# amberxie88/latent_diffusion_planning

Measured on AMD Instinct MI355X. Metric: latent plans/sec (horizon=9, 100 DDIM steps), higher is better.
Workload: dtype f32; 1 GPU; configs[1]: rm_lift planner ConditionalUnet1D (D=25, T=8, down_dims [256,512,1024]), 100-step DDIM, batch 256 synthetic latents per GPU, random-init weights, Philox noise, hipGraph-captured loop; plans_per_gpu=256, denoise_steps=100, sampler=ddim, graph=True, parallelism=dp1, ranks_seen_by_backend=1, backend=none, range_fallback=0, fp16_plane_launches=0

## Files before the change

### latent_diffusion_planning_amd/csrc/tconv.hpp

```cpp
#pragma once
#include <hip/hip_runtime.h>
#include <stdint.h>
#include <type_traits>

#pragma clang fp contract(off)

#ifndef LDP_W_NT
#define LDP_W_NT 0
#endif
#ifndef LDP_SPLIT_NPROD
#define LDP_SPLIT_NPROD 6
#endif
#ifndef LDP_S16_LF
#define LDP_S16_LF 100
#endif
#ifndef LDP_F16_MINW
#define LDP_F16_MINW 2
#endif
#ifndef LDP_RANGE_GUARD
#define LDP_RANGE_GUARD 1
#endif
#ifndef LDP_KERNARG_TOUCH
#define LDP_KERNARG_TOUCH 1
#endif
#ifndef LDP_KERNARG_PRELOAD
#define LDP_KERNARG_PRELOAD 1
#endif

namespace ldp {

typedef float f32x4 __attribute__((ext_vector_type(4)));

enum : int { MODE_K5 = 0, MODE_DOWN = 1, MODE_UP = 2, MODE_P1 = 3,
             MODE_K3H = 4,
             MODE_K3S = 5 };

enum : int {
  EP_GN = 1,
  EP_FILM = 2,
  EP_RESIN = 4,
  EP_RELU = 8,
  EP_STEP = 16,
  EP_EPSOUT = 32,
};

struct StepCoef {
  float t, inv_sqrt_ab, sqrt_1mab, c_x0, c_x, c_eps, sigma, pad;
};

constexpr int KW_MAX = 8;

struct ConvArgs {
  const float* xa;
  const float* xb;
  int ca, cb;
  const float* w;
  const float* bias;
  const float* bres;
  float* res_out;
  const float* gn_scale;
  const float* gn_bias;
  const float* film_t;
  const float* film_g;
  int film_stride;
  const int* k_dev;
  int k;
  const float* res_in;
  float* out;
  int B, cout, flags;
  int d_real;
  int rows_valid;
  StepCoef coef;
  const float* noise;
  const uint64_t* seed;
  int step;
  float* eps_out;
  int dbg;
  int cs;
  unsigned long long* xchg;
  int kw;
  unsigned long long* kw_slab;
  int kw_slot;
  const uint64_t* ctl;
  unsigned int* fault;
  int h_out, w_tiles, h_in, w_in;
  int ca_real;
  int by_sample;
  float* stats_part;
  int sb_qs;
  unsigned long long* tl;
};

#ifdef LDP_ABLATE
#define LDP_ABL(bit) ((a.dbg & (bit)) != 0)
#else
#define LDP_ABL(bit) (false)
#endif

#ifdef LDP_TIMELINE
#define LDP_TL(i)                                                                                         \
  do {                                                                                                    \
    if (a.tl) {                                                                                           \
      const unsigned long long t_ = (i) == 0 ? ldp_t_entry : __builtin_amdgcn_s_memtime();                \
      if (lane == 0)                                                                                      \
        a.tl[((size_t)(blockIdx.x + gridDim.x * (blockIdx.y + gridDim.y * blockIdx.z)) * 16 + wave) * 8 + (i)] = t_; \
    }                                                                                                     \
  } while (0)
#else
#define LDP_TL(i) do { } while (0)
#endif

__host__ __device__ constexpr int mode_taps(int mode) {
  return mode == MODE_K5 ? 5 : (mode == MODE_DOWN || mode == MODE_K3H || mode == MODE_K3S) ? 3
       : mode == MODE_UP ? 4 : 1;
}
__host__ __device__ constexpr bool mode_2d(int mode) { return mode == MODE_K3H || mode == MODE_K3S; }
__host__ __device__ constexpr int mode_ti(int mode, int to) {
  return mode == MODE_DOWN ? 2 * to : mode == MODE_UP ? to / 2 : mode == MODE_K3H ? to + 2
       : mode == MODE_K3S ? 2 * to + 2 : to;
}
__host__ __device__ constexpr int tap_src(int mode, int to, int j) {
  if (mode == MODE_K5) return to + j - 2;
  if (mode == MODE_DOWN || mode == MODE_K3S) return 2 * to + j;
  if (mode == MODE_K3H) return to + j;
  if (mode == MODE_UP) {
    const int q = to >> 1;
    if ((to & 1) == 0) return j == 0 ? q - 1 : (j == 2 ? q : -1);
    return j == 1 ? q : (j == 3 ? q + 1 : -1);
  }
  return j == 0 ? to : -1;
}
__host__ __device__ constexpr int tap_dst(int mode, int to_n, int ti, int j) {
  for (int to = 0; to < to_n; ++to)
    if (tap_src(mode, to, j) == ti) return to;
  return -1;
}
__host__ __device__ constexpr bool tap_used(int mode, int to_n, int j) {
  const int ti_n = mode_ti(mode, to_n);
  for (int to = 0; to < to_n; ++to) {
    const int ti = tap_src(mode, to, j);
    if (ti >= 0 && ti < ti_n) return true;
  }
  return false;
}
__host__ __device__ constexpr int valid_pairs(int mode, int to_n) {
  const int ti_n = mode_ti(mode, to_n);
  int n = 0;
  for (int to = 0; to < to_n; ++to)
    for (int j = 0; j < mode_taps(mode); ++j) {
      const int ti = tap_src(mode, to, j);
      if (ti >= 0 && ti < ti_n) ++n;
    }
  return n;
}

__device__ __forceinline__ int swz(int row, int slot) { return slot ^ ((4 - (row >> 2)) & 3); }

#ifndef LDP_EPILOGUE_IEEE
#define LDP_EPILOGUE_IEEE 0
#endif
__device__ __forceinline__ float mish_f(float x) {
#if LDP_EPILOGUE_IEEE
  const float e = expf(fminf(x, 20.0f));
  const float n = e * (e + 2.0f);
  return x * (n / (n + 2.0f));
#else
  const float e = __builtin_amdgcn_exp2f(fminf(x, 20.0f) * 1.4426950408889634f);
  const float n = e * (e + 2.0f);
  return x * (n * __builtin_amdgcn_rcpf(n + 2.0f));
#endif
}

template <int CTRL, int ROW_MASK>
__device__ __forceinline__ float dpp_add(float v) {
  return v + __int_as_float(__builtin_amdgcn_update_dpp(0, __float_as_int(v), CTRL, ROW_MASK, 0xF, false));
}
__device__ __forceinline__ float wave_sum(float v) {
  v = dpp_add<0xB1, 0xF>(v);
  v = dpp_add<0x4E, 0xF>(v);
  v = dpp_add<0x114, 0xF>(v);
  v = dpp_add<0x118, 0xF>(v);
  v = dpp_add<0x142, 0xA>(v);
  v = dpp_add<0x143, 0xC>(v);
  return __int_as_float(__builtin_amdgcn_readlane(__float_as_int(v), 63));
}

__device__ __forceinline__ unsigned long long granule_pack(unsigned int tag, float v) {
  const unsigned int b = __float_as_uint(v);
  return ((unsigned long long)(tag ^ b) << 32) | b;
}
typedef unsigned int u32x4_t __attribute__((ext_vector_type(4)));
constexpr int AUX_SC1 = 16;

__device__ __forceinline__ bool granule_ok(unsigned long long g, unsigned int tag) {
  return ((unsigned int)(g >> 32) ^ (unsigned int)g) == tag;
}

__device__ __forceinline__ void philox4x32_10(uint64_t seed, uint64_t elem, uint32_t step, uint32_t stream,
                                              uint32_t (&out)[4]) {
  uint32_t c0 = (uint32_t)elem, c1 = (uint32_t)(elem >> 32), c2 = step, c3 = stream;
  uint32_t k0 = (uint32_t)seed, k1 = (uint32_t)(seed >> 32);
#pragma unroll
  for (int r = 0; r < 10; ++r) {
    const uint64_t p0 = (uint64_t)0xD2511F53u * c0;
    const uint64_t p1 = (uint64_t)0xCD9E8D57u * c2;
    const uint32_t n0 = (uint32_t)(p1 >> 32) ^ c1 ^ k0;
    const uint32_t n1 = (uint32_t)p1;
    const uint32_t n2 = (uint32_t)(p0 >> 32) ^ c3 ^ k1;
    const uint32_t n3 = (uint32_t)p0;
    c0 = n0; c1 = n1; c2 = n2; c3 = n3;
    k0 += 0x9E3779B9u; k1 += 0xBB67AE85u;
  }
  out[0] = c0; out[1] = c1; out[2] = c2; out[3] = c3;
}

__device__ __forceinline__ float philox_normal(uint64_t seed, uint64_t elem, uint32_t step,
                                               uint32_t stream) {
  uint32_t w[4];
  philox4x32_10(seed, elem, step, stream, w);
  const float u1 = ((float)(w[0] >> 8) + 0.5f) * (1.0f / 16777216.0f);
  const float u2 = ((float)(w[1] >> 8) + 0.5f) * (1.0f / 16777216.0f);
  return sqrtf(-2.0f * logf(u1)) * cosf(6.28318530717958647692f * u2);
}

__host__ __device__ constexpr int mode_flag_mask(int mode) {
  return mode == MODE_K5 ? (EP_GN | EP_FILM | EP_RESIN)
       : mode == MODE_P1 ? (EP_RESIN | EP_RELU | EP_STEP | EP_EPSOUT)
       : mode_2d(mode) ? EP_RESIN : 0;
}
__host__ __device__ constexpr int mode_flag_forced(int mode) { return mode == MODE_K5 ? EP_GN : 0; }

template <int MODE, int TO, int NWN, int KS, int CPI, int MB = 1, int SPLIT = 0>
struct TConvCfg {
  static constexpr int TI = mode_ti(MODE, TO);
  static constexpr int NJ = mode_taps(MODE);
  static constexpr bool S32 = (SPLIT == 1 || SPLIT == 4) && MB == 2;
  static constexpr bool S16 = (SPLIT == 1 && MB == 1) || SPLIT == 2 || SPLIT == 3;
  static constexpr bool F16 = SPLIT == 3 || SPLIT == 4;
  static constexpr int NPL = F16 ? 2 : 3;
  static constexpr int NWC = S32 ? NWN / 2 : NWN;
  static constexpr int NW = NWC * KS;
  static constexpr int NT = 64 * NW;
  static constexpr int BN = 16 * NWN;
  static constexpr int BNP = BN + 4;
  static constexpr int NC = KS * CPI;
  static constexpr int CH_IT = 16 * NC;
  static constexpr int XT = MB * TI * NC * 256 * (SPLIT ? NPL : 2) / 2;
  static constexpr int NLD = (MB * TI * NC * 64) / NT;
  static constexpr int EPI = MB * KS * TO * 16 * BNP;
  static constexpr int TILE_FLOATS = (2 * XT > EPI) ? 2 * XT : EPI;
  static constexpr bool STATS = MODE == MODE_K3H && BN == 64 && MB == 1 && (NW == 8 || NW == 4);
  static constexpr int LDS_FLOATS = TILE_FLOATS + (STATS ? 2 * NW * 64 : 0);
  static constexpr int LDS_BYTES = LDS_FLOATS * 4;
  static constexpr int EPL = (TO * BN) / 64;
  static_assert((MB * TI * NC * 64) % NT == 0, "staging loads must divide evenly");
  static_assert((TO * BN) % 64 == 0, "epilogue needs TO*BN multiple of 64");
  static_assert(NW <= 16, "at most 16 waves");
  static_assert(!SPLIT || (S32 && MODE == MODE_K5 && NWN % 2 == 0) || (S16 && (MODE == MODE_K5 || MODE == MODE_DOWN || MODE == MODE_UP || ((MODE == MODE_K3S || MODE == MODE_K3H) && SPLIT == 3 && MB == 1)) && MB <= 2 && CPI % 2 == 0),
                "split operands: 32-sample x 32-column wave tiles (SPLIT = 1, MB = 2, k = 5) or 16 x 16 tiles over 32-channel steps (MB = 1, or SPLIT = 2 with MB = 2; k = 5, stride-2, transposed)");
};

struct ConvHot {
  static __host__ __device__ int pack(const ConvArgs& a, bool zfold) {
    return (a.cs & 15) | ((a.kw & 15) << 4) | ((a.by_sample & 1) << 8) | ((a.sb_qs & 15) << 9) | ((zfold ? 1 : 0) << 13) | (((a.by_sample >> 1) & 1) << 14);
  }
};
#if LDP_KERNARG_PRELOAD
#define LDP_KERNEL_PARAMS const float* h_xa, const float* h_xb, const float* h_w, int h_B, int h_ca, int h_cb, int h_cout, \
                          int h_ca_real, int h_pk, int h_dbg, const ConvArgs a_in
#define LDP_KERNEL_ARGS(a, zfold) (a).xa, (a).xb, (a).w, (a).B, (a).ca, (a).cb, (a).cout, (a).ca_real, ConvHot::pack(a, zfold), (a).dbg, (a)
#else
#define LDP_KERNEL_PARAMS const ConvArgs a
#define LDP_KERNEL_ARGS(a, zfold) (a)
#endif

typedef __bf16 bf16x8_t __attribute__((ext_vector_type(8)));
typedef float f32x16 __attribute__((ext_vector_type(16)));
__device__ __forceinline__ void split4(const f32x4 v, uint2& h, uint2& m, uint2& l) {
  unsigned short hh[4], mm[4], ll[4];
#pragma unroll
  for (int i = 0; i < 4; ++i) {
    const __bf16 bh = (__bf16)v[i];
    const float r1 = v[i] - (float)bh;
    const __bf16 bm = (__bf16)r1;
    const float r2 = r1 - (float)bm;
    const __bf16 bl = (__bf16)r2;
    hh[i] = __builtin_bit_cast(unsigned short, bh); mm[i] = __builtin_bit_cast(unsigned short, bm); ll[i] = __builtin_bit_cast(unsigned short, bl);
  }
  h = uint2{(unsigned)hh[0] | ((unsigned)hh[1] << 16), (unsigned)hh[2] | ((unsigned)hh[3] << 16)};
  m = uint2{(unsigned)mm[0] | ((unsigned)mm[1] << 16), (unsigned)mm[2] | ((unsigned)mm[3] << 16)};
  l = uint2{(unsigned)ll[0] | ((unsigned)ll[1] << 16), (unsigned)ll[2] | ((unsigned)ll[3] << 16)};
}

typedef _Float16 f16x8_t __attribute__((ext_vector_type(8)));
__device__ __forceinline__ void split4h(const f32x4 v, uint2& h, uint2& l) {
  unsigned short hh[4], ll[4];
#pragma unroll
  for (int i = 0; i < 4; ++i) {
    const _Float16 bh = (_Float16)v[i];
    const _Float16 bl = (_Float16)((v[i] - (float)bh) * 2048.0f);
    hh[i] = __builtin_bit_cast(unsigned short, bh); ll[i] = __builtin_bit_cast(unsigned short, bl);
  }
  h = uint2{(unsigned)hh[0] | ((unsigned)hh[1] << 16), (unsigned)hh[2] | ((unsigned)hh[3] << 16)};
  l = uint2{(unsigned)ll[0] | ((unsigned)ll[1] << 16), (unsigned)ll[2] | ((unsigned)ll[3] << 16)};
}

template <int MODE, int TO, int NWN, int KS, int CPI, bool RES_OUT, int MB = 1, bool KWS = false, int SPLIT = 0>
__global__ __launch_bounds__(64 * (((SPLIT == 1 || SPLIT == 4) && MB == 2) ? NWN / 2 : NWN) * KS,
                              (SPLIT == 3 && (NWN * KS == 4 || (NWN * KS == 8 && KS >= 2 && NWN <= 4 && (!RES_OUT || TO == 2)) || (NWN == 2 && KS == 4)) && TO <= 8 && !(TO == 8 && RES_OUT)) ? LDP_F16_MINW : 1) void tconv_kernel(LDP_KERNEL_PARAMS) {
#if LDP_KERNARG_PRELOAD
  ConvArgs a = a_in;
  a.xa = h_xa; a.xb = h_xb; a.w = h_w; a.B = h_B; a.ca = h_ca; a.cb = h_cb; a.cout = h_cout; a.ca_real = h_ca_real;
  a.cs = h_pk & 15; a.kw = (h_pk >> 4) & 15; a.by_sample = (h_pk >> 8) & 1; a.sb_qs = (h_pk >> 9) & 15; a.dbg = h_dbg;
#endif
  using C = TConvCfg<MODE, TO, NWN, KS, CPI, MB, SPLIT>;
  constexpr int TI = C::TI, NJ = C::NJ, NC = C::NC, NT = C::NT, BN = C::BN, BNP = C::BNP;
  static_assert(!RES_OUT || MODE == MODE_K5, "RES_OUT only for k=5 convs");
  static_assert(!SPLIT || !KWS, "split operands: no K split over work-groups");
  constexpr bool S32 = C::S32, S16 = C::S16;

  extern __shared__ f32x4 smem4[];
  float* smem = reinterpret_cast<float*>(smem4);

#ifdef LDP_TIMELINE
  const unsigned long long ldp_t_entry = __builtin_amdgcn_s_memtime();
#endif
#if LDP_KERNARG_TOUCH && !LDP_KERNARG_PRELOAD
  asm volatile("" ::"s"(a.xa), "s"(a.gn_bias), "s"(a.B), "s"(a.seed), "s"(a.ctl));
#endif
  const int tid = threadIdx.x, lane = tid & 63;
  const int wave = __builtin_amdgcn_readfirstlane(tid >> 6);
  const int wn = wave % C::NWC, ks = wave / C::NWC;
  const int cs = a.cs > 1 ? a.cs : 1;
  const int ngroups = a.by_sample ? gridDim.z : gridDim.x;
  int grp = a.by_sample ? blockIdx.z : blockIdx.x;
  const int kw = (KWS && a.kw > 1) ? a.kw : 1;
  const int half = blockIdx.y & (cs - 1);
  const int kpart = (blockIdx.y >> (cs >> 1)) & (kw - 1);
#if LDP_KERNARG_PRELOAD
  int sb = a.by_sample ? blockIdx.x : blockIdx.z;
  if ((h_pk >> 13) & 1) sb += gridDim.z * (blockIdx.y >> ((cs >> 1) + (__ffs(kw) - 1)));
#else
  int sb = a.by_sample ? blockIdx.x : blockIdx.z + gridDim.z * (blockIdx.y >> ((cs >> 1) + (__ffs(kw) - 1)));
#endif
  if (MODE == MODE_P1 && a.by_sample && a.sb_qs > 0) {
    const int xcd = blockIdx.x & 7, j = blockIdx.x >> 3;
    sb = ((((j >> a.sb_qs) << 3) + xcd) << a.sb_qs) + (j & ((1 << a.sb_qs) - 1));
  }
#if LDP_KERNARG_PRELOAD
  if constexpr (SPLIT != 0) {
    if ((h_pk >> 14) & 1) {
      const int X = grp, si = sb;
      grp = (X >> 2) + 2 * (si & 3);
      sb = (X & 3) + 4 * (si >> 2);
    }
  }
#endif
  if (sb * (16 * MB) >= a.B) return;
  const int cbk = grp * cs + half;
  const int b0 = sb * (16 * MB);
  const int r = lane & 15, kq = lane >> 4;
  const int nblk_total = S32 ? a.cout >> 5 : a.cout >> 4;
  const int nblk = cbk * C::NWC + wn;
  const int cin = a.ca + a.cb;
  int nit_all = LDP_ABL(8) ? 0 : (mode_2d(MODE) ? 3 * cin : cin) / C::CH_IT;
  if constexpr (MODE == MODE_K5 && RES_OUT && SPLIT == 0 && !KWS) {
    if (a.ca_real > 0 && !LDP_ABL(8)) nit_all = (a.ca_real + C::CH_IT - 1) / C::CH_IT;
  }
  const int it0 = kpart * (nit_all / kw);
  const int nit = it0 + nit_all / kw;
  if LDP_ABL(64) return;
  LDP_TL(0);

  f32x4 acc[MB][TO];
  f32x4 racc[MB][RES_OUT ? TO : 1];
  f32x4 acc_lo[C::F16 ? MB : 1][C::F16 ? TO : 1], racc_lo[C::F16 ? MB : 1][C::F16 && RES_OUT ? TO : 1];
#pragma unroll
  for (int m = 0; m < (C::F16 ? MB : 1); ++m) {
#pragma unroll
    for (int t = 0; t < (C::F16 ? TO : 1); ++t) acc_lo[m][t] = f32x4{0.f, 0.f, 0.f, 0.f};
#pragma unroll
    for (int t = 0; t < (C::F16 && RES_OUT ? TO : 1); ++t) racc_lo[m][t] = f32x4{0.f, 0.f, 0.f, 0.f};
  }
#pragma unroll
  for (int m = 0; m < MB; ++m) {
#pragma unroll
    for (int t = 0; t < TO; ++t) acc[m][t] = f32x4{0.f, 0.f, 0.f, 0.f};
#pragma unroll
    for (int t = 0; t < (RES_OUT ? TO : 1); ++t) racc[m][t] = f32x4{0.f, 0.f, 0.f, 0.f};
  }

  int st_goff[C::NLD];
  int st_loff[C::NLD];
  int st_cc[C::NLD];
  int st_mask[mode_2d(MODE) ? C::NLD : 1];
#pragma unroll
  for (int i = 0; i < C::NLD; ++i) {
    const int idx = tid + i * NT;
    const int q = idx & 3;
    const int cc = (idx >> 2) % NC;
    const int rr = (idx / (4 * NC)) & 15;
    const int tm = idx / (64 * NC);
    const int tt = tm % TI, mb = tm / TI;
    st_cc[i] = cc * 16 + q * 4;
    const int bb = (b0 + mb * 16 + rr) < a.B ? (b0 + mb * 16 + rr) : (a.B - 1);
    st_goff[i] = bb * TI + tt;
    st_loff[i] = (((mb * TI + tt) * NC + cc) * 16 + rr) * 16 + swz(rr, q) * 4;
    if constexpr (S32) st_loff[i] = (((tt * NC + cc) * C::NPL) * 64 + (q >> 1) * 32 + mb * 16 + rr) * 4 + (q & 1) * 2;
    if constexpr (S16) st_loff[i] = ((((mb * TI + tt) * (NC / 2) + (cc >> 1)) * C::NPL) * 64 + ((cc & 1) * 2 + (q >> 1)) * 16 + rr) * 4 + (q & 1) * 2;
    if (mode_2d(MODE)) {
      const int wt = bb % a.w_tiles, hh = (bb / a.w_tiles) % a.h_out, n = bb / (a.w_tiles * a.h_out);
      const int w = MODE == MODE_K3H ? wt * TO - 1 + tt : 2 * wt * TO + tt;
      const int h0 = MODE == MODE_K3H ? hh - 1 : 2 * hh;
      const bool wok = w >= 0 && w < a.w_in;
      int m = 0;
#pragma unroll
      for (int dh = 0; dh < 3; ++dh) m |= (wok && h0 + dh >= 0 && h0 + dh < a.h_in) ? (1 << dh) : 0;
      st_mask[i] = m;
      st_goff[i] = (n * a.h_in + h0) * a.w_in + w;
    }
  }

  f32x4 xst[C::NLD];
  auto stage_load = [&](int it) {
    const int c0 = it * C::CH_IT;
    if (mode_2d(MODE)) {
      const int dh = c0 / a.ca, cbase = c0 - dh * a.ca;
#pragma unroll
      for (int i = 0; i < C::NLD; ++i) {
        const bool ok = (st_mask[i] >> dh) & 1;
        const int pix = ok ? st_goff[i] + dh * a.w_in : 0;
        const f32x4 v = *reinterpret_cast<const f32x4*>(a.xa + (size_t)pix * a.ca + cbase + st_cc[i]);
        xst[i] = ok ? v : f32x4{0.f, 0.f, 0.f, 0.f};
      }
      return;
    }
    const bool second = (c0 >= a.ca);
    const float* base = second ? a.xb : a.xa;
    const int cw = second ? a.cb : a.ca;
    const int cbase = second ? c0 - a.ca : c0;
    const int creal = a.ca_real > 0 ? a.ca_real : 0x7fffffff;
    const int stride = a.ca_real > 0 ? a.ca_real : cw;
#pragma unroll
    for (int i = 0; i < C::NLD; ++i) {
      const bool ok = (cbase + st_cc[i]) < creal;
      xst[i] = *reinterpret_cast<const f32x4*>(base + (size_t)st_goff[i] * stride + (ok ? cbase + st_cc[i] : 0));
    }
  };
  auto stage_store = [&](float* buf) {
    if constexpr (C::F16) {
#pragma unroll
      for (int i = 0; i < C::NLD; ++i) {
        uint2 ph, pl;
        split4h(xst[i], ph, pl);
        *reinterpret_cast<uint2*>(buf + st_loff[i]) = ph;
        *reinterpret_cast<uint2*>(buf + st_loff[i] + 256) = pl;
      }
      return;
    }
    if constexpr (SPLIT) {
#pragma unroll
      for (int i = 0; i < C::NLD; ++i) {
        uint2 ph, pm, pl;
        split4(xst[i], ph, pm, pl);
        *reinterpret_cast<uint2*>(buf + st_loff[i]) = ph;
        *reinterpret_cast<uint2*>(buf + st_loff[i] + 256) = pm;
        *reinterpret_cast<uint2*>(buf + st_loff[i] + 512) = pl;
      }
      return;
    }
#pragma unroll
    for (int i = 0; i < C::NLD; ++i) *reinterpret_cast<f32x4*>(buf + st_loff[i]) = xst[i];
  };

  constexpr bool SKIPZ = MODE == MODE_K5 && RES_OUT && SPLIT == 0 && TO >= 8 && KS > 1;
  constexpr int NJW = NJ + (RES_OUT ? 1 : 0);
  constexpr int NSTEP = S16 ? CPI / 2 : 1;
  constexpr int WCH = S16 ? 1 : CPI;
  constexpr int RN = RES_OUT ? WCH : 1;
  constexpr int WPL = SPLIT ? C::NPL : 1;
  f32x4 wb0[NJ][WCH * WPL], wb1[NJ][WCH * WPL];
  f32x4 rb0[RN * WPL], rb1[RN * WPL];
  auto wload = [&](int it, f32x4 (&b)[NJ][WCH * WPL], f32x4 (&rb)[RN * WPL]) {
#pragma unroll
    for (int ci = 0; ci < WCH; ++ci) {
      const int gc = S16 ? (it / NSTEP) * (NC / 2) + ks * NSTEP + (it % NSTEP) : it * NC + ks * CPI + ci;
#pragma unroll
      for (int j = 0; j < NJ; ++j) {
        if constexpr (SPLIT) {
          if (tap_used(MODE, TO, j)) {
#pragma unroll
            for (int pl = 0; pl < WPL; ++pl) {
              const size_t off = ((((size_t)gc * NJW + j) * nblk_total + nblk) * WPL + pl) * 256 + lane * 4;
              b[j][ci * WPL + pl] = *reinterpret_cast<const f32x4*>(a.w + off);
            }
          }
        } else
        if (tap_used(MODE, TO, j)) {
          const size_t off = (((size_t)gc * NJW + j) * nblk_total + nblk) * 256 + lane * 4;
          b[j][ci] = (LDP_W_NT && KWS) ? __builtin_nontemporal_load(reinterpret_cast<const f32x4*>(a.w + off))
                                       : *reinterpret_cast<const f32x4*>(a.w + off);
        }
      }
      if constexpr (RES_OUT && SPLIT) {
#pragma unroll
        for (int pl = 0; pl < WPL; ++pl) {
          const size_t off = ((((size_t)gc * NJW + NJ) * nblk_total + nblk) * WPL + pl) * 256 + lane * 4;
          rb[ci * WPL + pl] = *reinterpret_cast<const f32x4*>(a.w + off);
        }
      } else
      if (RES_OUT) {
        const size_t off = (((size_t)gc * NJW + NJ) * nblk_total + nblk) * 256 + lane * 4;
        rb[ci] = (LDP_W_NT && KWS) ? __builtin_nontemporal_load(reinterpret_cast<const f32x4*>(a.w + off))
                                   : *reinterpret_cast<const f32x4*>(a.w + off);
      }
    }
  };

  f32x16 acc32[S32 ? TO : 1], racc32[S32 && RES_OUT ? TO : 1];
  f32x16 acc32_lo[S32 && C::F16 ? TO : 1], racc32_lo[S32 && C::F16 && RES_OUT ? TO : 1];
  if constexpr (S32 && C::F16) {
#pragma unroll
    for (int t = 0; t < TO; ++t)
#pragma unroll
      for (int i = 0; i < 16; ++i) acc32_lo[t][i] = 0.f;
#pragma unroll
    for (int t = 0; t < (RES_OUT ? TO : 1); ++t)
#pragma unroll
      for (int i = 0; i < 16; ++i) racc32_lo[t][i] = 0.f;
  }
  if constexpr (S32) {
#pragma unroll
    for (int t = 0; t < TO; ++t)
#pragma unroll
      for (int i = 0; i < 16; ++i) acc32[t][i] = 0.f;
#pragma unroll
    for (int t = 0; t < (RES_OUT ? TO : 1); ++t)
#pragma unroll
      for (int i = 0; i < 16; ++i) racc32[t][i] = 0.f;
  }
  auto iteration = [&](auto last_tag, int it, f32x4 (&bc)[NJ][WCH * WPL], f32x4 (&rc)[RN * WPL], f32x4 (&bl)[NJ][WCH * WPL],
                       f32x4 (&rl)[RN * WPL]) {
    constexpr bool LAST = decltype(last_tag)::value;
    float* xcur = smem + (it & 1) * C::XT;
    float* xnext = smem + ((it + 1) & 1) * C::XT;
    const int itn = LDP_ABL(256) ? it0 : (LAST || (it + 1) < nit) ? it + 1 : it;
    if (!LAST) {
      if (!(SPLIT && LDP_ABL(2048))) stage_load(itn);
      if (!S16 && !(SPLIT && LDP_ABL(1024))) wload(itn, bl, rl);
    }
    if constexpr (S16) {
      constexpr int NPAIR = valid_pairs(MODE, TO) + (RES_OUT ? TO : 0);
      constexpr int NUSED = (tap_used(MODE, TO, 0) ? 1 : 0) + (NJ > 1 && tap_used(MODE, TO, 1) ? 1 : 0) + (NJ > 2 && tap_used(MODE, TO, 2) ? 1 : 0) +
                            (NJ > 3 && tap_used(MODE, TO, 3) ? 1 : 0) + (NJ > 4 && tap_used(MODE, TO, 4) ? 1 : 0);
      constexpr int NPL = C::NPL;
      constexpr int NWL = (NUSED + (RES_OUT ? 1 : 0)) * NPL;
      constexpr int NMFMA = (C::F16 ? 3 : LDP_SPLIT_NPROD) * NPAIR * MB;
      constexpr int NREAD = MB * TI * NPL;
      constexpr int AHEAD = MB * (TI > 2 ? 2 : TI) * NPL;
      auto step = [&](auto pc_tag, f32x4 (&wc)[NJ][WCH * WPL], f32x4 (&rcur)[RN * WPL], f32x4 (&wn)[NJ][WCH * WPL], f32x4 (&rnext)[RN * WPL]) {
        constexpr int pc = decltype(pc_tag)::value;
        constexpr bool PREF = pc + 1 < NSTEP || !LAST;
        if (PREF && !LDP_ABL(1024)) wload(pc + 1 < NSTEP ? it * NSTEP + pc + 1 : itn * NSTEP, wn, rnext);
        f32x4 asp[MB][TI][NPL];
#pragma unroll
        for (int ti = 0; ti < TI; ++ti) {
#pragma unroll
          for (int m = 0; m < MB; ++m)
#pragma unroll
            for (int pl = 0; pl < NPL; ++pl)
              asp[m][ti][pl] = *reinterpret_cast<const f32x4*>(xcur + (((((m * TI + ti) * (NC / 2) + ks * NSTEP + pc) * NPL + pl) * 64 + lane) * 4));
        }
        if constexpr (C::F16) {
          constexpr int FA[3] = {1, 0, 0}, FB[3] = {0, 1, 0};
#pragma unroll
          for (int ti = 0; ti < TI; ++ti) {
#pragma unroll
            for (int pi = 0; pi < 3; ++pi) {
#pragma unroll
              for (int j = 0; j <= NJ; ++j) {
                if (j == NJ && !RES_OUT) continue;
                const int to = j == NJ ? (ti < TO ? ti : -1) : tap_dst(MODE, TO, ti, j < NJ ? j : 0);
                if (to < 0) continue;
                const f32x4* bp = j == NJ ? &rcur[0] : &wc[j < NJ ? j : 0][0];
                const f16x8_t bv = __builtin_bit_cast(f16x8_t, bp[FB[pi]]);
#pragma unroll
                for (int m = 0; m < MB; ++m) {
                  const f16x8_t av = __builtin_bit_cast(f16x8_t, asp[m][ti][FA[pi]]);
                  f32x4& dst = j == NJ ? (pi < 2 ? racc_lo[m][RES_OUT ? to : 0] : racc[m][RES_OUT ? to : 0]) : (pi < 2 ? acc_lo[m][to] : acc[m][to]);
                  dst = __builtin_amdgcn_mfma_f32_16x16x32_f16(av, bv, dst, 0, 0, 0);
                }
              }
            }
          }
        } else {
        constexpr int NP = LDP_SPLIT_NPROD;
        constexpr int PA9[9] = {2, 1, 2, 1, 2, 0, 1, 0, 0}, PB9[9] = {2, 2, 1, 1, 0, 2, 0, 1, 0};
#pragma unroll
        for (int ti = 0; ti < TI; ++ti) {
#pragma unroll
          for (int pi = 9 - NP; pi < 9; ++pi) {
#pragma unroll
            for (int j = 0; j <= NJ; ++j) {
              if (j == NJ && !RES_OUT) continue;
              const int to = j == NJ ? (ti < TO ? ti : -1) : tap_dst(MODE, TO, ti, j < NJ ? j : 0);
              if (to < 0) continue;
              const f32x4* bp = j == NJ ? &rcur[0] : &wc[j < NJ ? j : 0][0];
              const bf16x8_t bv = __builtin_bit_cast(bf16x8_t, bp[PB9[pi]]);
#pragma unroll
              for (int m = 0; m < MB; ++m) {
                const bf16x8_t av = __builtin_bit_cast(bf16x8_t, asp[m][ti][PA9[pi]]);
                if (j == NJ) racc[m][RES_OUT ? to : 0] = __builtin_amdgcn_mfma_f32_16x16x32_bf16(av, bv, racc[m][RES_OUT ? to : 0], 0, 0, 0);
                else acc[m][to] = __builtin_amdgcn_mfma_f32_16x16x32_bf16(av, bv, acc[m][to], 0, 0, 0);
              }
            }
          }
        }
        }
        {
          constexpr int NLOADS = (PREF ? NWL : 0) + ((pc == 0 && !LAST) ? C::NLD : 0);
          constexpr int NRD = NREAD - AHEAD;
          constexpr int ML = NMFMA * LDP_S16_LF / 100 > 0 ? NMFMA * LDP_S16_LF / 100 : 1;
#pragma unroll
          for (int i = 0; i < AHEAD; ++i) __builtin_amdgcn_sched_group_barrier(0x100, 1, 0);
#pragma unroll
          for (int m = 0; m < NMFMA; ++m) {
            if (NLOADS > 0 && m < ML) {
              const int nl = (m + 1) * NLOADS / ML - m * NLOADS / ML;
              if (nl > 0) __builtin_amdgcn_sched_group_barrier(0x020, 1, 0);
              if (nl > 1) __builtin_amdgcn_sched_group_barrier(0x020, 1, 0);
              if (nl > 2) __builtin_amdgcn_sched_group_barrier(0x020, 1, 0);
            }
            if (NRD > 0 && (m + 1) * NRD / NMFMA != m * NRD / NMFMA) __builtin_amdgcn_sched_group_barrier(0x100, 1, 0);
            __builtin_amdgcn_sched_group_barrier(0x008, 1, 0);
          }
        }
      };
      step(std::integral_constant<int, 0>{}, bc, rc, bl, rl);
      if constexpr (NSTEP > 1) step(std::integral_constant<int, 1>{}, bl, rl, bc, rc);
      if constexpr (NSTEP > 2) step(std::integral_constant<int, 2>{}, bc, rc, bl, rl);
      if constexpr (NSTEP > 3) step(std::integral_constant<int, 3>{}, bl, rl, bc, rc);
      static_assert(NSTEP <= 4, "at most four 32-channel steps per iteration");
      if (LDP_ABL(512)) return;
      if (!LAST) stage_store(xnext);
      __syncthreads();
      return;
    }
    if constexpr (S32) {
      constexpr int NPL = C::NPL;
      f32x4 asp[TI][CPI][NPL];
#pragma unroll
      for (int ti = 0; ti < TI; ++ti)
#pragma unroll
        for (int ci = 0; ci < CPI; ++ci)
#pragma unroll
          for (int pl = 0; pl < NPL; ++pl)
            asp[ti][ci][pl] = *reinterpret_cast<const f32x4*>(xcur + ((((ti * NC + ks * CPI + ci) * NPL + pl) * 64 + lane) * 4));
      auto pair = [&](const f32x4* ap, const f32x4* bp, f32x16& c, f32x16& clo) {
        if constexpr (C::F16) {
          const f16x8_t ah = __builtin_bit_cast(f16x8_t, ap[0]), al = __builtin_bit_cast(f16x8_t, ap[1]);
          const f16x8_t bh = __builtin_bit_cast(f16x8_t, bp[0]), bl2 = __builtin_bit_cast(f16x8_t, bp[1]);
          clo = __builtin_amdgcn_mfma_f32_32x32x16_f16(al, bh, clo, 0, 0, 0);
          c = __builtin_amdgcn_mfma_f32_32x32x16_f16(ah, bh, c, 0, 0, 0);
          clo = __builtin_amdgcn_mfma_f32_32x32x16_f16(ah, bl2, clo, 0, 0, 0);
        } else {
          const bf16x8_t ah = __builtin_bit_cast(bf16x8_t, ap[0]), am = __builtin_bit_cast(bf16x8_t, ap[1]), al = __builtin_bit_cast(bf16x8_t, ap[NPL - 1]);
          const bf16x8_t bh = __builtin_bit_cast(bf16x8_t, bp[0]), bm = __builtin_bit_cast(bf16x8_t, bp[1]), bl2 = __builtin_bit_cast(bf16x8_t, bp[NPL - 1]);
          c = __builtin_amdgcn_mfma_f32_32x32x16_bf16(am, bm, c, 0, 0, 0);
          c = __builtin_amdgcn_mfma_f32_32x32x16_bf16(al, bh, c, 0, 0, 0);
          c = __builtin_amdgcn_mfma_f32_32x32x16_bf16(ah, bl2, c, 0, 0, 0);
          c = __builtin_amdgcn_mfma_f32_32x32x16_bf16(am, bh, c, 0, 0, 0);
          c = __builtin_amdgcn_mfma_f32_32x32x16_bf16(ah, bm, c, 0, 0, 0);
          c = __builtin_amdgcn_mfma_f32_32x32x16_bf16(ah, bh, c, 0, 0, 0);
        }
      };
#pragma unroll
      for (int ci = 0; ci < CPI; ++ci)
#pragma unroll
        for (int j = 0; j < NJ; ++j)
#pragma unroll
          for (int to = 0; to < TO; ++to) {
            const int ti = tap_src(MODE, to, j);
            if (ti >= 0 && ti < TI) pair(&asp[ti][ci][0], &bc[j][ci * WPL], acc32[to], acc32_lo[C::F16 ? to : 0]);
          }
      if constexpr (RES_OUT) {
#pragma unroll
        for (int ci = 0; ci < CPI; ++ci)
#pragma unroll
          for (int to = 0; to < TO; ++to) pair(&asp[to][ci][0], &rc[ci * WPL], racc32[to], racc32_lo[C::F16 ? to : 0]);
      }
      {
        constexpr int NUSED = (tap_used(MODE, TO, 0) ? 1 : 0) + (NJ > 1 && tap_used(MODE, TO, 1) ? 1 : 0) + (NJ > 2 && tap_used(MODE, TO, 2) ? 1 : 0) +
                              (NJ > 3 && tap_used(MODE, TO, 3) ? 1 : 0) + (NJ > 4 && tap_used(MODE, TO, 4) ? 1 : 0);
        constexpr int NLOADS = LAST ? 0 : C::NLD + (NUSED + (RES_OUT ? 1 : 0)) * CPI * C::NPL;
        constexpr int NMFMA = CPI * (C::F16 ? 3 : 6) * (valid_pairs(MODE, TO) + (RES_OUT ? TO : 0));
        constexpr int MPL = NMFMA / (NLOADS > 0 ? NLOADS : 1) > 0 ? NMFMA / (NLOADS > 0 ? NLOADS : 1) : 1;
#pragma unroll
        for (int i = 0; i < TI * CPI * C::NPL; ++i) __builtin_amdgcn_sched_group_barrier(0x100, 1, 0);
#pragma unroll
        for (int i = 0; i < NLOADS; ++i) {
          __builtin_amdgcn_sched_group_barrier(0x020, 1, 0);
          __builtin_amdgcn_sched_group_barrier(0x008, MPL, 0);
        }
        if (NMFMA - NLOADS * MPL > 0) __builtin_amdgcn_sched_group_barrier(0x008, NMFMA - NLOADS * MPL, 0);
      }
      if (!LAST) stage_store(xnext);
      __syncthreads();
      return;
    }
    f32x4 areg[MB][TI][CPI];
#pragma unroll
    for (int m = 0; m < MB; ++m)
#pragma unroll
      for (int ti = 0; ti < TI; ++ti)
#pragma unroll
        for (int ci = 0; ci < CPI; ++ci)
          areg[m][ti][ci] = *reinterpret_cast<const f32x4*>(
              xcur + (((m * TI + ti) * NC + ks * CPI + ci) * 16 + r) * 16 + swz(r, kq) * 4);

    const bool dead_slice = SKIPZ && a.ca_real > 0 && (it * C::CH_IT + ks * CPI * 16) >= a.ca_real;
    if (!dead_slice) {
#pragma unroll
    for (int ci = 0; ci < CPI; ++ci) {
#pragma unroll
      for (int s = 0; s < 4; ++s) {
#pragma unroll
        for (int j = 0; j < NJ; ++j) {
#pragma unroll
          for (int to = 0; to < TO; ++to) {
            const int ti = tap_src(MODE, to, j);
            if (ti >= 0 && ti < TI) {
#pragma unroll
              for (int m = 0; m < MB; ++m)
                acc[m][to] = __builtin_amdgcn_mfma_f32_16x16x4f32(areg[m][ti][ci][s], bc[j][ci][s],
                                                                  acc[m][to], 0, 0, 0);
            }
          }
        }
        if (RES_OUT) {
#pragma unroll
          for (int to = 0; to < TO; ++to)
#pragma unroll
            for (int m = 0; m < MB; ++m)
              racc[m][to] = __builtin_amdgcn_mfma_f32_16x16x4f32(areg[m][to][ci][s], rc[ci][s],
                                                                 racc[m][to], 0, 0, 0);
        }
      }
    }
    }
    if (LAST) {
#pragma unroll
      for (int i = 0; i < MB * TI * CPI; ++i) __builtin_amdgcn_sched_group_barrier(0x100, 1, 0);
    } else {
      constexpr int NUSED = (tap_used(MODE, TO, 0) ? 1 : 0) + (NJ > 1 && tap_used(MODE, TO, 1) ? 1 : 0) +
                            (NJ > 2 && tap_used(MODE, TO, 2) ? 1 : 0) + (NJ > 3 && tap_used(MODE, TO, 3) ? 1 : 0) +
                            (NJ > 4 && tap_used(MODE, TO, 4) ? 1 : 0);
      constexpr int NLOADS = C::NLD + (NUSED + (RES_OUT ? 1 : 0)) * CPI;
      constexpr int NMFMA = MB * CPI * 4 * (valid_pairs(MODE, TO) + (RES_OUT ? TO : 0));
      constexpr int MPL = NMFMA / NLOADS > 0 ? NMFMA / NLOADS : 1;
#pragma unroll
      for (int i = 0; i < MB * TI * CPI; ++i) __builtin_amdgcn_sched_group_barrier(0x100, 1, 0);
#pragma unroll
      for (int i = 0; i < NLOADS; ++i) {
        __builtin_amdgcn_sched_group_barrier(0x020, 1, 0);
        __builtin_amdgcn_sched_group_barrier(0x008, MPL, 0);
      }
      if (NMFMA - NLOADS * MPL > 0) __builtin_amdgcn_sched_group_barrier(0x008, NMFMA - NLOADS * MPL, 0);
      __builtin_amdgcn_sched_group_barrier(0x200, C::NLD, 0);
    }
    if (!LAST) stage_store(xnext);
    __syncthreads();
  };

  stage_load(it0);
  wload(S16 ? it0 * NSTEP : it0, wb0, rb0);
  stage_store(smem + (it0 & 1) * C::XT);
  __syncthreads();
  LDP_TL(1);

  if (mode_2d(MODE) && !S16) {
    for (int it = it0; it < nit; it += 2) {
      iteration(std::false_type{}, it, wb0, rb0, wb1, rb1);
      if (it + 1 < nit) iteration(std::false_type{}, it + 1, wb1, rb1, wb0, rb0);
    }
  } else {
    int it = it0;
    if constexpr (S16 && NSTEP % 2 == 0) {
      for (; it + 1 < nit; ++it) iteration(std::false_type{}, it, wb0, rb0, wb1, rb1);
      iteration(std::true_type{}, it, wb0, rb0, wb1, rb1);
    } else {
    for (; it + 2 < nit; it += 2) {
      iteration(std::false_type{}, it, wb0, rb0, wb1, rb1);
      iteration(std::false_type{}, it + 1, wb1, rb1, wb0, rb0);
    }
    if (it + 2 == nit) {
      iteration(std::false_type{}, it, wb0, rb0, wb1, rb1);
      iteration(std::true_type{}, it + 1, wb1, rb1, wb0, rb0);
    } else if (it + 1 == nit) {
      iteration(std::true_type{}, it, wb0, rb0, wb1, rb1);
    }
    }
  }

  if constexpr (C::F16 && S32) {
#pragma unroll
    for (int t = 0; t < TO; ++t)
#pragma unroll
      for (int i = 0; i < 16; ++i) acc32[t][i] = acc32[t][i] + acc32_lo[t][i] * (1.0f / 2048.0f);
    if constexpr (RES_OUT) {
#pragma unroll
      for (int t = 0; t < TO; ++t)
#pragma unroll
        for (int i = 0; i < 16; ++i) racc32[t][i] = racc32[t][i] + racc32_lo[t][i] * (1.0f / 2048.0f);
    }
  }
  if constexpr (C::F16 && !S32) {
#pragma unroll
    for (int m = 0; m < MB; ++m) {
#pragma unroll
      for (int t = 0; t < TO; ++t) acc[m][t] = acc[m][t] + acc_lo[m][t] * (1.0f / 2048.0f);
      if constexpr (RES_OUT) {
#pragma unroll
        for (int t = 0; t < TO; ++t) racc[m][t] = racc[m][t] + racc_lo[m][t] * (1.0f / 2048.0f);
      }
    }
  }
  LDP_TL(2);
  if LDP_ABL(16) return;
  const int ecol = wn * 16 + (lane & 15);
  const int erow0 = (lane >> 4) * 4;
  const int flags = (a.flags & mode_flag_mask(MODE)) | mode_flag_forced(MODE);
  constexpr int EPL = C::EPL;
  constexpr int NS = 16 * MB;
  constexpr int SPW = (NS + C::NW - 1) / C::NW;
  constexpr bool FULL = (NS % C::NW) == 0;
  const unsigned lane_to = BN <= 64 ? (unsigned)lane / BN : 0u;
  const unsigned lane_col = BN <= 64 ? (unsigned)lane % BN : (unsigned)lane;
  auto e_to = [](int e) { return BN <= 64 ? e * (64 / BN) : e / (BN / 64); };
  auto e_col = [](int e) { return BN <= 64 ? 0 : 64 * (e % (BN / 64)); };
  const unsigned lane_chan = (unsigned)(cbk * BN) + lane_col;
  const unsigned lane_eoff = __umul24(lane_to, (unsigned)a.cout) + lane_chan;
  const unsigned lane_uoff = __umul24(lane_to, (unsigned)a.d_real) + lane_chan;
  float p_bias[EPL], p_gs[EPL], p_gb[EPL], p_rb[EPL];
  float p_fts[SPW][EPL], p_fgs[SPW][EPL], p_ftb[SPW][EPL], p_fgb[SPW][EPL], p_add[SPW][EPL], p_nz[SPW][EPL];
#pragma unroll
  for (int e = 0; e < EPL; ++e) {
    p_bias[e] = (a.bias + e_col(e))[lane_chan];
    p_gs[e] = (flags & EP_GN) ? (a.gn_scale + e_col(e))[lane_chan] : 1.0f;
    p_gb[e] = (flags & EP_GN) ? (a.gn_bias + e_col(e))[lane_chan] : 0.0f;
    p_rb[e] = RES_OUT ? (a.bres + e_col(e))[lane_chan] : 0.0f;
  }
  const bool f_film = (flags & EP_FILM) != 0, f_res = (flags & EP_RESIN) != 0;
  const bool f_step = (flags & EP_STEP) != 0;
#pragma unroll
  for (int si = 0; si < SPW; ++si)
#pragma unroll
    for (int e = 0; e < EPL; ++e) p_fts[si][e] = p_fgs[si][e] = p_ftb[si][e] = p_fgb[si][e] = p_add[si][e] = p_nz[si][e] = 0.0f;
  if (f_film) {
#pragma unroll
    for (int si = 0; si < SPW; ++si) {
      const int sr = wave + si * C::NW;
      const int b = (b0 + sr) < a.B ? (b0 + sr) : (a.B - 1);
      int kk = a.k;
      if (a.k_dev) kk = a.k_dev[b];
      const float* ft = a.film_t + (size_t)kk * a.film_stride;
      const float* fg = a.film_g + (size_t)b * a.film_stride;
#pragma unroll
      for (int e = 0; e < EPL; ++e) {
        p_fts[si][e] = (ft + e_col(e))[lane_chan];
        p_fgs[si][e] = (fg + e_col(e))[lane_chan];
        p_ftb[si][e] = (ft + a.cout + e_col(e))[lane_chan];
        p_fgb[si][e] = (fg + a.cout + e_col(e))[lane_chan];
      }
    }
  }
  if (f_res || f_step) {
    const float* rp = f_res ? a.res_in : a.out;
#pragma unroll
    for (int si = 0; si < SPW; ++si) {
      const int sr = wave + si * C::NW;
      const int b = (b0 + sr) < a.B ? (b0 + sr) : (a.B - 1);
#pragma unroll
      for (int e = 0; e < EPL; ++e)
        p_add[si][e] = (rp + ((size_t)b * TO + e_to(e)) * a.cout + e_col(e))[lane_eoff];
    }
  }
  if (f_step && a.noise && a.coef.sigma != 0.f) {
#pragma unroll
    for (int si = 0; si < SPW; ++si) {
      const int sr = wave + si * C::NW;
      const int b = (b0 + sr) < a.B ? (b0 + sr) : (a.B - 1);
#pragma unroll
      for (int e = 0; e < EPL; ++e) {
        const int to = (int)lane_to + e_to(e), c = (int)lane_chan + e_col(e);
        if (c < a.d_real && (b * TO + to) < a.rows_valid)
          p_nz[si][e] = (a.noise + ((size_t)b * TO + e_to(e)) * a.d_real + e_col(e))[lane_uoff];
      }
    }
  }

  {
    constexpr int pass = 0;
    if constexpr (S32) {
#pragma unroll
      for (int to = 0; to < TO; ++to)
#pragma unroll
        for (int i = 0; i < 16; ++i) {
          const int row32 = (i & 3) + 8 * (i >> 2) + 4 * (lane >> 5);
          smem[((((row32 >> 4) * KS + ks) * TO + to) * 16 + (row32 & 15)) * BNP + wn * 32 + (lane & 31)] = acc32[to][i];
        }
    } else
#pragma unroll
    for (int m = 0; m < MB; ++m) {
#pragma unroll
      for (int to = 0; to < TO; ++to) {
#pragma unroll
        for (int i = 0; i < 4; ++i)
          smem[(((m * KS + ks) * TO + to) * 16 + erow0 + i) * BNP + ecol] = acc[m][to][i];
      }
    }
    __syncthreads();
    LDP_TL(3);

    constexpr int TILE = NS * TO * BN;
    constexpr bool KW_OK = KWS && (MODE == MODE_K5 || MODE == MODE_DOWN || MODE == MODE_UP) && MB == 1 && TO * BN <= 512;
    unsigned long long* kw_tile = nullptr;
    unsigned int ktag = 0;
    if (KW_OK && kw > 1) {
      const int tile_id = sb * (ngroups * cs) + cbk;
      kw_tile = a.kw_slab + (size_t)(tile_id * kw) * (2 * TILE);
      ktag = (((unsigned int)a.ctl[2] & 0xfffu) << 20) | (((unsigned int)a.step + 1u) << 6) | (unsigned int)a.kw_slot;
      if (kpart != 0) {
        unsigned long long* mine = kw_tile + (size_t)kpart * (2 * TILE);
#pragma unroll
        for (int pass = 0; pass < (RES_OUT ? 2 : 1); ++pass) {
          if (pass == 1) {
            __syncthreads();
#pragma unroll
            for (int to = 0; to < TO; ++to)
#pragma unroll
              for (int i = 0; i < 4; ++i)
                smem[((ks * TO + to) * 16 + erow0 + i) * BNP + ecol] = racc[0][RES_OUT ? to : 0][i];
            __syncthreads();
          }
          const auto krsrc = __builtin_amdgcn_make_buffer_rsrc(mine, 0, 0x7ffffff0, 0x00020000);
          constexpr int PAIRS = TO * BN / 2;
#pragma unroll
          for (int si = 0; si < SPW; ++si) {
            const int sr = wave + si * C::NW;
            if (!FULL && sr >= NS) continue;
#pragma unroll
            for (int pc = 0; pc < (PAIRS + 63) / 64; ++pc) {
              if (PAIRS < 64 && lane >= PAIRS) continue;
              const int el = 2 * (lane + 64 * pc);
              const int to = el / BN, col = el % BN;
              float x0 = 0.0f, x1 = 0.0f;
#pragma unroll
              for (int k2 = 0; k2 < KS; ++k2) {
                x0 += smem[((k2 * TO + to) * 16 + sr) * BNP + col];
                x1 += smem[((k2 * TO + to) * 16 + sr) * BNP + col + 1];
              }
              const unsigned long long g0 = granule_pack(ktag, x0), g1 = granule_pack(ktag, x1);
              const u32x4_t gv = {(unsigned int)g0, (unsigned int)(g0 >> 32), (unsigned int)g1, (unsigned int)(g1 >> 32)};
              __builtin_amdgcn_raw_buffer_store_b128(gv, krsrc, (unsigned int)((pass * TILE + sr * (TO * BN) + el) * 8), 0, AUX_SC1);
            }
          }
        }
        return;
      }
    }
    auto kw_add = [&](float x, int pass, int sr, int el) {
      if (!(KW_OK && kw > 1)) return x;
      unsigned long long pv[KW_MAX - 1];
      int spin = 0;
      for (;;) {
        bool ok = true;
#pragma unroll
        for (int q = 0; q < KW_MAX - 1; ++q) {
          pv[q] = 0;
          if (q + 1 < kw)
            pv[q] = __hip_atomic_load(kw_tile + (size_t)(q + 1) * (2 * TILE) + pass * TILE + sr * (TO * BN) + el,
                                      __ATOMIC_RELAXED, __HIP_MEMORY_SCOPE_AGENT);
        }
        asm volatile("s_waitcnt vmcnt(0)" ::: "memory");
#pragma unroll
        for (int q = 0; q < KW_MAX - 1; ++q) ok = ok && (q + 1 >= kw || granule_ok(pv[q], ktag));
        if (__all(ok)) break;
        if (++spin > (1 << 18) || ((spin & 1023) == 0 && __hip_atomic_load(a.fault, __ATOMIC_RELAXED, __HIP_MEMORY_SCOPE_SYSTEM) != 0u)) {
          if (lane == 0) *a.fault = 1u;
          break;
        }
        __builtin_amdgcn_s_sleep(1);
      }
#pragma unroll
      for (int q = 0; q < KW_MAX - 1; ++q) x += (q + 1 < kw) ? __uint_as_float((unsigned int)pv[q]) : 0.0f;
      return x;
    };

    const bool xch = (cs > 1) && (flags & EP_GN) && !LDP_ABL(32);
    const auto xrsrc = __builtin_amdgcn_make_buffer_rsrc(const_cast<unsigned long long*>(a.xchg), 0, 0x7ffffff0, 0x00020000);
    unsigned int xbase = 0;
    unsigned int tag = 0;
    if (xch) {
      xbase = (unsigned int)((sb * MB * ngroups + grp) * 4) * 256u;
      tag = ((unsigned int)a.ctl[2] << 12) + (unsigned int)a.step + 1u;
    }
    float vv[SPW][EPL];
    float s1a[SPW], s2a[SPW];
    bool range_bad = false;
#pragma unroll
    for (int si = 0; si < SPW; ++si) {
      const int sr = wave + si * C::NW;
      float s1 = 0.f, s2 = 0.f;
#pragma unroll
      for (int e = 0; e < EPL; ++e) {
        const int el = lane + 64 * e;
        const int to = el / BN, col = el % BN;
        float x = p_bias[e];
        if (FULL || sr < NS) {
#pragma unroll
          for (int k2 = 0; k2 < KS; ++k2)
            x += smem[((((sr >> 4) * KS + k2) * TO + to) * 16 + (sr & 15)) * BNP + col];
          x = kw_add(x, 0, sr, el);
        }
        vv[si][e] = x;
        s1 += x;
        s2 += x * x;
      }
      if (flags & EP_GN) {
        s1 = wave_sum(s1);
        s2 = wave_sum(s2);
        if (xch && (FULL || sr < NS) && lane == 0) {
          const unsigned long long g1 = granule_pack(tag, s1), g2 = granule_pack(tag, s2);
          const u32x4_t gv = {(unsigned int)g1, (unsigned int)(g1 >> 32), (unsigned int)g2, (unsigned int)(g2 >> 32)};
          __builtin_amdgcn_raw_buffer_store_b128(gv, xrsrc, xbase + (unsigned int)(((sr >> 4) * ngroups * 4 + half) * 256 + (sr & 15) * 16), 0, AUX_SC1);
        }
      }
      if constexpr (C::F16) {
        if (LDP_RANGE_GUARD) range_bad = range_bad || !(s2 <= 3.0e38f);
      }
      s1a[si] = s1;
      s2a[si] = s2;
    }

    LDP_TL(4);
    if (RES_OUT) {
      __syncthreads();
      if constexpr (S32) {
#pragma unroll
        for (int to = 0; to < TO; ++to)
#pragma unroll
          for (int i = 0; i < 16; ++i) {
            const int row32 = (i & 3) + 8 * (i >> 2) + 4 * (lane >> 5);
            smem[((((row32 >> 4) * KS + ks) * TO + to) * 16 + (row32 & 15)) * BNP + wn * 32 + (lane & 31)] = racc32[RES_OUT ? to : 0][i];
          }
      } else
#pragma unroll
      for (int m = 0; m < MB; ++m) {
#pragma unroll
        for (int to = 0; to < TO; ++to) {
#pragma unroll
          for (int i = 0; i < 4; ++i)
            smem[(((m * KS + ks) * TO + to) * 16 + erow0 + i) * BNP + ecol] = racc[m][RES_OUT ? to : 0][i];
        }
      }
      __syncthreads();
#pragma unroll
      for (int si = 0; si < SPW; ++si) {
        const int sr = wave + si * C::NW;
        const int b = b0 + sr;
        if ((!FULL && sr >= NS) || b >= a.B) continue;
#pragma unroll
        for (int e = 0; e < EPL; ++e) {
          const int el = lane + 64 * e;
          const int to = el / BN, col = el % BN;
          float x = p_rb[e];
#pragma unroll
          for (int k2 = 0; k2 < KS; ++k2)
            x += smem[((((sr >> 4) * KS + k2) * TO + to) * 16 + (sr & 15)) * BNP + col];
          x = kw_add(x, 1, sr, el);
          if (!LDP_ABL(128) || x == 12345.f) (a.res_out + ((size_t)b * TO + e_to(e)) * a.cout + e_col(e))[lane_eoff] = x;
        }
      }
    }

    LDP_TL(5);
    float gs1 = 0.f, gs2 = 0.f;
#pragma unroll
    for (int si = 0; si < SPW; ++si) {
      const int sr = wave + si * C::NW;
      if (!FULL && sr >= NS) continue;
      const int b = b0 + sr;
      const bool live = b < a.B;
      float* v = vv[si];
      float mean = 0.f, rstd = 1.f;
      if (flags & EP_GN) {
        float s1 = s1a[si], s2 = s2a[si];
        if (xch) {
          u32x4_t pg[3];
          int spin = 0;
          for (;;) {
#pragma unroll
            for (int q = 0; q < 3; ++q) {
              pg[q] = u32x4_t{0u, 0u, 0u, 0u};
              if (q < cs - 1) {
                const int pp = q < half ? q : q + 1;
                pg[q] = __builtin_amdgcn_raw_buffer_load_b128(xrsrc, xbase + (unsigned int)(((sr >> 4) * ngroups * 4 + pp) * 256 + (sr & 15) * 16), 0, AUX_SC1);
              }
            }
            asm volatile("s_waitcnt vmcnt(0)" : "+v"(pg[0]), "+v"(pg[1]), "+v"(pg[2]) :: "memory");
            bool ok = true;
#pragma unroll
            for (int q = 0; q < 3; ++q)
              ok = ok && (q >= cs - 1 || (((pg[q][0] ^ pg[q][1]) == tag) && ((pg[q][2] ^ pg[q][3]) == tag)));
            if (ok) break;
            if (++spin > (1 << 20) || ((spin & 1023) == 0 && __hip_atomic_load(a.fault, __ATOMIC_RELAXED, __HIP_MEMORY_SCOPE_SYSTEM) != 0u)) {
              if (lane == 0) *a.fault = 1u;
              break;
            }
            __builtin_amdgcn_s_sleep(1);
          }
#ifdef LDP_TIMELINE
          if (a.tl && lane == 0) {
            atomicAdd(&a.tl[120000], 1ull);
            atomicAdd(&a.tl[120001], (unsigned long long)spin);
          }
#endif
          float t1 = 0.f, t2 = 0.f;
#pragma unroll
          for (int pp = 0; pp < 4; ++pp) {
            if (pp >= cs) continue;
            const int q = pp < half ? pp : pp - 1;
            float p1 = s1, p2 = s2;
            if (pp != half) {
              p1 = __uint_as_float(q == 0 ? pg[0][0] : q == 1 ? pg[1][0] : pg[2][0]);
              p2 = __uint_as_float(q == 0 ? pg[0][2] : q == 1 ? pg[1][2] : pg[2][2]);
            }
            t1 = pp == 0 ? p1 : t1 + p1;
            t2 = pp == 0 ? p2 : t2 + p2;
          }
          s1 = t1;
          s2 = t2;
        }
        const float inv_n = 1.0f / (float)(TO * BN * cs);
        mean = s1 * inv_n;
        const float var = fmaxf(s2 * inv_n - mean * mean, 0.0f);
#if LDP_EPILOGUE_IEEE
        rstd = 1.0f / sqrtf(var + 1e-6f);
#else
        rstd = __builtin_amdgcn_rsqf(var + 1e-6f);
#endif
      }
      if (!live) continue;
#pragma unroll
      for (int e = 0; e < EPL; ++e) {
        const int el = lane + 64 * e;
        const int to = el / BN, col = el % BN;
        const int c = cbk * BN + col;
        float y = v[e];
        if (flags & EP_GN) {
          y = (y - mean) * rstd * p_gs[e] + p_gb[e];
          y = mish_f(y);
        }
        if (flags & EP_FILM) y = (p_fts[si][e] + p_fgs[si][e]) * y + (p_ftb[si][e] + p_fgb[si][e]);
        float* const optr = a.out + ((size_t)b * TO + e_to(e)) * a.cout + e_col(e);
        if (flags & EP_RESIN) y += p_add[si][e];
        if (flags & EP_RELU) y = fmaxf(y, 0.0f);
        if (flags & (EP_STEP | EP_EPSOUT)) {
          if (c < a.d_real && (b * TO + to) < a.rows_valid) {
            if (flags & EP_EPSOUT) (a.eps_out + ((size_t)b * TO + e_to(e)) * a.d_real + e_col(e))[lane_uoff] = y;
            if (flags & EP_STEP) {
              const float xt = p_add[si][e];
              float z = 0.f;
              if (a.coef.sigma != 0.f) {
                if (a.noise) z = p_nz[si][e];
                else z = philox_normal(a.seed[0], (a.seed[1] + (uint64_t)(b * TO + to)) * (uint64_t)a.cout
                                       + (uint64_t)c, (uint32_t)a.step, 0u);
              }
              float x0 = (xt - a.coef.sqrt_1mab * y) * a.coef.inv_sqrt_ab;
              x0 = fminf(fmaxf(x0, -1.0f), 1.0f);
              optr[lane_eoff] = a.coef.c_x0 * x0 + a.coef.c_x * xt + a.coef.c_eps * y + a.coef.sigma * z;
            }
          }
        } else if (!LDP_ABL(128) || y == 12345.f) {
          optr[lane_eoff] = y;
          if (C::STATS) { gs1 += y; gs2 += y * y; }
        }
      }
    }
    if constexpr (C::F16) {
      if (LDP_RANGE_GUARD && range_bad && a.fault) a.fault[1] = 1u;
    }
    LDP_TL(6);
#ifdef LDP_TIMELINE
    if (a.tl) { asm volatile("s_waitcnt vmcnt(0)" ::: "memory"); LDP_TL(7); }
#endif
    if (C::STATS) {
      if (a.stats_part) {
        float* sp = smem + C::TILE_FLOATS;
        sp[wave * 64 + lane] = gs1;
        sp[(C::NW + wave) * 64 + lane] = gs2;
        __syncthreads();
        if (tid < 128) {
          const int which = tid >> 6, c = tid & 63;
          float t = 0.f;
#pragma unroll
          for (int w = 0; w < C::NW; ++w) t += sp[(which * C::NW + w) * 64 + c];
          a.stats_part[((size_t)sb * a.cout + cbk * BN + c) * 2 + which] = t;
        }
      }
    }
  }
}

__host__ __device__ constexpr bool tconv_kw_ok(int mode, int to, int nwn, int mb) {
  return (mode == MODE_K5 || mode == MODE_DOWN || mode == MODE_UP) && mb == 1 && to * 16 * nwn <= 512;
}

struct ConvPlan {
  int mode, to, nwn, ks, cpi, res_out;
  int mb = 1;
  int kws = 0;
  int split = 0;
  int bn() const { return 16 * nwn; }
  int chunk() const { return 16 * ks * cpi; }
};
int tconv_launch(const ConvPlan& p, const ConvArgs& a, hipStream_t stream);
int tconv_init_all();
int tconv_init_k5();
int tconv_init_k5r();
int tconv_init_misc();
int tconv_init_2d();
int tconv_launch_2d(const ConvPlan& p, const ConvArgs& a, hipStream_t stream);
int tconv_launch_k5(const ConvPlan& p, const ConvArgs& a, hipStream_t stream);
int tconv_launch_k5r(const ConvPlan& p, const ConvArgs& a, hipStream_t stream);
int tconv_launch_misc(const ConvPlan& p, const ConvArgs& a, hipStream_t stream);
int tconv_launch_split(const ConvPlan& p, const ConvArgs& a, hipStream_t stream);
int tconv_init_split();

}
```

Measured before the change: 5394 plans/s.

## Load only own first-stage slice into LDS and store outputs with SC1 cache hint

For non-split 1D convs with one N-wave, each wave now loads only its own K-slice of the first input stage straight into shared memory and skips the initial barrier, instead of running the cooperative stage_load/store plus __syncthreads. Separately, residual and main epilogue stores go through raw buffer stores carrying an SC1 cache-policy bit instead of plain global stores. The aim is to shorten the kernel prologue and change cache behaviour for outputs the next kernel consumes. Dropping the barrier relies on each wave reading only the LDS slice it wrote, and the buffer descriptor uses a fixed large range with no bounds checking beyond that.

Measured after the change: 5429 plans/s (median of 6 runs). No clear change (+0.7%).

```diff
diff --git a/latent_diffusion_planning_amd/csrc/tconv.hpp b/latent_diffusion_planning_amd/csrc/tconv.hpp
--- a/latent_diffusion_planning_amd/csrc/tconv.hpp
+++ b/latent_diffusion_planning_amd/csrc/tconv.hpp
@@ -22,6 +22,12 @@
 #endif
 #ifndef LDP_KERNARG_TOUCH
 #define LDP_KERNARG_TOUCH 1
+#endif
+#ifndef LDP_OWN_FIRST
+#define LDP_OWN_FIRST 1
+#endif
+#ifndef LDP_OUT_SC1
+#define LDP_OUT_SC1 1
 #endif
 #ifndef LDP_KERNARG_PRELOAD
 #define LDP_KERNARG_PRELOAD 1
@@ -318,6 +324,8 @@
   static_assert(!RES_OUT || MODE == MODE_K5, "RES_OUT only for k=5 convs");
   static_assert(!SPLIT || !KWS, "split operands: no K split over work-groups");
   constexpr bool S32 = C::S32, S16 = C::S16;
+  constexpr bool OWN_FIRST = LDP_OWN_FIRST && SPLIT == 0 && !mode_2d(MODE) && NWN == 1;
+  constexpr bool OUT_SC1 = LDP_OUT_SC1 && SPLIT == 0 && !mode_2d(MODE);
 
   extern __shared__ f32x4 smem4[];
   float* smem = reinterpret_cast<float*>(smem4);
@@ -772,10 +780,44 @@
     __syncthreads();
   };
 
-  stage_load(it0);
-  wload(S16 ? it0 * NSTEP : it0, wb0, rb0);
-  stage_store(smem + (it0 & 1) * C::XT);
-  __syncthreads();
+  if constexpr (OWN_FIRST) {
+    wload(it0, wb0, rb0);
+    constexpr int NOWN = MB * TI * CPI;
+    f32x4 xo[NOWN];
+    const int orr = lane >> 2, oq = lane & 3;
+    const int c0 = it0 * C::CH_IT;
+    const bool second = (c0 >= a.ca);
+    const float* base = second ? a.xb : a.xa;
+    const int cw = second ? a.cb : a.ca;
+    const int cbase = second ? c0 - a.ca : c0;
+    const int creal = a.ca_real > 0 ? a.ca_real : 0x7fffffff;
+    const int stride = a.ca_real > 0 ? a.ca_real : cw;
+#pragma unroll
+    for (int m = 0; m < MB; ++m) {
+      const int bb = (b0 + m * 16 + orr) < a.B ? (b0 + m * 16 + orr) : (a.B - 1);
+#pragma unroll
+      for (int tt = 0; tt < TI; ++tt)
+#pragma unroll
+        for (int ci = 0; ci < CPI; ++ci) {
+          const int cch = (ks * CPI + ci) * 16 + oq * 4;
+          const bool ok = (cbase + cch) < creal;
+          xo[(m * TI + tt) * CPI + ci] = *reinterpret_cast<const f32x4*>(base + (size_t)(bb * TI + tt) * stride + (ok ? cbase + cch : 0));
+        }
+    }
+    float* buf = smem + (it0 & 1) * C::XT;
+#pragma unroll
+    for (int m = 0; m < MB; ++m)
+#pragma unroll
+      for (int tt = 0; tt < TI; ++tt)
+#pragma unroll
+        for (int ci = 0; ci < CPI; ++ci)
+          *reinterpret_cast<f32x4*>(buf + (((m * TI + tt) * NC + ks * CPI + ci) * 16 + orr) * 16 + swz(orr, oq) * 4) = xo[(m * TI + tt) * CPI + ci];
+  } else {
+    stage_load(it0);
+    wload(S16 ? it0 * NSTEP : it0, wb0, rb0);
+    stage_store(smem + (it0 & 1) * C::XT);
+    __syncthreads();
+  }
   LDP_TL(1);
 
   if (mode_2d(MODE) && !S16) {
@@ -1079,7 +1121,14 @@
           for (int k2 = 0; k2 < KS; ++k2)
             x += smem[((((sr >> 4) * KS + k2) * TO + to) * 16 + (sr & 15)) * BNP + col];
           x = kw_add(x, 1, sr, el);
-          if (!LDP_ABL(128) || x == 12345.f) (a.res_out + ((size_t)b * TO + e_to(e)) * a.cout + e_col(e))[lane_eoff] = x;
+          if (!LDP_ABL(128) || x == 12345.f) {
+            float* const rptr = a.res_out + ((size_t)b * TO + e_to(e)) * a.cout + e_col(e);
+            if constexpr (OUT_SC1)
+              __builtin_amdgcn_raw_buffer_store_b32(__float_as_uint(x), __builtin_amdgcn_make_buffer_rsrc(rptr, 0, 0x7ffffff0, 0x00020000),
+                                                    lane_eoff * 4u, 0, AUX_SC1);
+            else
+              rptr[lane_eoff] = x;
+          }
         }
       }
     }
@@ -1183,7 +1232,11 @@
             }
           }
         } else if (!LDP_ABL(128) || y == 12345.f) {
-          optr[lane_eoff] = y;
+          if constexpr (OUT_SC1)
+            __builtin_amdgcn_raw_buffer_store_b32(__float_as_uint(y), __builtin_amdgcn_make_buffer_rsrc(optr, 0, 0x7ffffff0, 0x00020000),
+                                                  lane_eoff * 4u, 0, AUX_SC1);
+          else
+            optr[lane_eoff] = y;
           if (C::STATS) { gs1 += y; gs2 += y * y; }
         }
       }
```
